# linhthi/BLISS-GNN

Measured on AMD Instinct MI355X. Metric: steps/sec (train step: sample_blocks + gather + SAGE fwd/bwd + Adam + exp3), reddit-like, higher is better.
Workload: dtype bf16

## Files before the change

bliss_gnn_amd/csrc/common.cuh:

```cuda
#pragma once
#include <hip/hip_runtime.h>
#include <stdint.h>
#include "bliss_gnn.h"

#define BLISS_WAVE 64

#define FRAC_DST 40
#define FRAC_SRC 44
#define FRAC_BLK 36

#define BLISS_ERR_CAP_FRONTIER 1
#define BLISS_ERR_CAP_CAND     2
#define BLISS_ERR_CAP_KEPT     4
#define BLISS_ERR_CAP_EDGES    8
#define BLISS_ERR_NONFINITE   16
#define BLISS_ERR_FIXED_RANGE 32
#define BLISS_ERR_CAP_SEEDS   64
#define BLISS_ERR_RNG_STREAM 128
#define BLISS_ERR_FLAG_TIMEOUT 256

typedef uint16_t bf16_t;

__device__ __forceinline__ float bf2f(bf16_t b) { return __uint_as_float(((uint32_t)b) << 16); }

// ... 53 lines not shown
__device__ __forceinline__ long long bf_to_fixed_wide(bf16_t b, int frac, long long* lo, int* sticky, int* bad) {
  uint32_t e = (b >> 7) & 0xff, m = b & 0x7f;
  if (e == 255) { *bad |= BLISS_ERR_NONFINITE; return 0; }
  if (e == 0) e = 1; else m |= 0x80;
  const int shift = (int)e - 134 + frac;
  const bool neg = (b & 0x8000) != 0;
  if (shift >= 0) {
    if (shift > 55) { *bad |= BLISS_ERR_FIXED_RANGE; return 0; }
    const long long mag = (long long)((uint64_t)m << shift);
    return neg ? -mag : mag;
  }
  const int rs = -shift;
  const uint32_t top = rs >= 8 ? 0u : (m >> rs);
  const uint32_t r = rs >= 8 ? m : (m & ((1u << rs) - 1u));
  if (r) {
    long long l;
    if (rs <= 40) l = (long long)((uint64_t)r << (40 - rs));
    else {
      const int d = rs - 40;
      l = d >= 8 ? 0 : (long long)(r >> d);
      if (d >= 8 || (r & ((1u << d) - 1u))) *sticky = 1;
    }
    *lo += neg ? -l : l;
  }
  return neg ? -(long long)top : (long long)top;
}

__device__ __forceinline__ bf16_t fixed_wide_to_bf(int64_t hi, int64_t lo, int sticky, int frac, int* bad) {
  if (lo == 0 && !sticky) return fixed_to_bf(hi, frac, bad);
  __int128 t = ((__int128)hi << 40) + (__int128)lo;
  if (t == 0) return 0;
  const uint32_t sign = t < 0 ? 0x8000u : 0u;
  const unsigned __int128 mag = t < 0 ? (unsigned __int128)(-t) : (unsigned __int128)t;
  const uint64_t mh = (uint64_t)(mag >> 64), ml = (uint64_t)mag;
  const int msb = mh ? 127 - __clzll((long long)mh) : 63 - __clzll((long long)ml);
  const int f = frac + 40;
  auto round_shift = [&](int sh) -> uint64_t {
    if (sh <= 0) return (uint64_t)(mag << (-sh));
    if (sh > 126) return 0;
    uint64_t q = (uint64_t)(mag >> sh);
    const unsigned __int128 rem = mag & ((((unsigned __int128)1) << sh) - 1), half = ((unsigned __int128)1) << (sh - 1);
    if (rem > half || (rem == half && (sticky || (q & 1)))) q += 1;
    return q;
  };
  if (msb - f + 127 <= 0) return (bf16_t)(sign | (uint32_t)round_shift(f - 133));
  uint64_t q = round_shift(msb - 7);
  int e = msb - f + 127;
  if (q >= 256) { q >>= 1; e += 1; }
  if (e >= 255) { *bad |= BLISS_ERR_FIXED_RANGE; return 0; }
  return (bf16_t)(sign | ((uint32_t)e << 7) | ((uint32_t)q & 0x7f));
}

struct PlainRange { unsigned lo, span; };
__device__ __forceinline__ PlainRange bf_plain_range(int frac) {
  int e_lo = 134 - frac, e_hi = 189 - frac;
  if (e_hi > 254) e_hi = 254;
  PlainRange r;
  r.lo = e_lo <= 1 ? 0u : (unsigned)e_lo << 7;
  const unsigned end = e_hi < 1 ? 0u : (unsigned)(e_hi + 1) << 7;
  r.span = end > r.lo ? end - r.lo : 0u;
  return r;
}
__device__ __forceinline__ bool bf_is_plain(bf16_t b, PlainRange r) { return (unsigned)b - r.lo < r.span; }
__device__ __forceinline__ long long bf_fixed_plain(bf16_t b, int frac) {
  const unsigned ef = (unsigned)b >> 7, m = (b & 0x7fu) | (ef ? 0x80u : 0u);
  const int shift = (int)(ef ? ef : 1u) - 134 + frac;
  return (long long)((uint64_t)m << (shift & 63));
}

__device__ __forceinline__ int lane_id() { return threadIdx.x & (BLISS_WAVE - 1); }

__device__ __forceinline__ int64_t shfl_up_i64(int64_t v, int d) {
  int lo = __shfl_up((int)(v & 0xffffffffll), d), hi = __shfl_up((int)(v >> 32), d);
  return ((int64_t)hi << 32) | (uint32_t)lo;
}

template <int CTRL, int ROW_MASK>
__device__ __forceinline__ int dpp_mov0(int v) { return __builtin_amdgcn_update_dpp(0, v, CTRL, ROW_MASK, 0xf, false); }
template <int CTRL, int ROW_MASK>
__device__ __forceinline__ long long dpp_mov0_i64(long long v) {
  const int lo = dpp_mov0<CTRL, ROW_MASK>((int)(v & 0xffffffffll)), hi = dpp_mov0<CTRL, ROW_MASK>((int)(v >> 32));
  return ((long long)hi << 32) | (unsigned)lo;
}
__device__ __forceinline__ int wave_total_i32(int v) {
  v += dpp_mov0<0x111, 0xf>(v); v += dpp_mov0<0x112, 0xf>(v); v += dpp_mov0<0x114, 0xf>(v); v += dpp_mov0<0x118, 0xf>(v);
  v += dpp_mov0<0x142, 0xa>(v); v += dpp_mov0<0x143, 0xc>(v);
  return __builtin_amdgcn_readlane(v, 63);
}
__device__ __forceinline__ int wave_max_u31(int v) {
  v = max(v, dpp_mov0<0x111, 0xf>(v)); v = max(v, dpp_mov0<0x112, 0xf>(v)); v = max(v, dpp_mov0<0x114, 0xf>(v));
  v = max(v, dpp_mov0<0x118, 0xf>(v)); v = max(v, dpp_mov0<0x142, 0xa>(v)); v = max(v, dpp_mov0<0x143, 0xc>(v));
  return __builtin_amdgcn_readlane(v, 63);
}
__device__ __forceinline__ int bf_exp_field(bf16_t b) { const int e = (b >> 7) & 0xff; return e == 0 ? 1 : e; }
__device__ __forceinline__ int rel_frac(int frac, int emax) { const int s = 126 - emax; return frac + (s > 0 ? s : 0); }

__device__ __forceinline__ long long wave_total_i64(long long v) {
  v += dpp_mov0_i64<0x111, 0xf>(v); v += dpp_mov0_i64<0x112, 0xf>(v); v += dpp_mov0_i64<0x114, 0xf>(v);
  v += dpp_mov0_i64<0x118, 0xf>(v); v += dpp_mov0_i64<0x142, 0xa>(v); v += dpp_mov0_i64<0x143, 0xc>(v);
  const int lo = __builtin_amdgcn_readlane((int)(v & 0xffffffffll), 63), hi = __builtin_amdgcn_readlane((int)(v >> 32), 63);
  return ((long long)hi << 32) | (unsigned)lo;
}
__device__ __forceinline__ bool wave_single_key(int key, int* k0) {
  const unsigned long long act = __ballot(key >= 0);
  if (!act) { *k0 = -1; return true; }
  *k0 = __builtin_amdgcn_readlane(key, __ffsll((long long)act) - 1);
  return __ballot(key >= 0 && key != *k0) == 0ull;
}

__device__ __forceinline__ void wave_segsum_atomic_i64(int key, int64_t v, unsigned long long* acc) {
  const int lane = lane_id();
  int k0;
  if (wave_single_key(key, &k0)) {
    if (k0 < 0) return;
    const long long tot = wave_total_i64(key >= 0 ? v : 0);
    if (lane == 0 && tot != 0) atomicAdd(acc + k0, (unsigned long long)tot);
    return;
  }
#pragma unroll
  for (int d = 1; d < BLISS_WAVE; d <<= 1) {
    int64_t vu = shfl_up_i64(v, d);
    int ku = __shfl_up(key, d);
    if (lane >= d && ku == key) v += vu;
  }
  int kn = __shfl_down(key, 1);
  if (key >= 0 && (lane == BLISS_WAVE - 1 || kn != key) && v != 0)
    atomicAdd(acc + key, (unsigned long long)v);
}
__device__ __forceinline__ void wave_segsum_atomic_i32(int key, int v, int* acc) {
  const int lane = lane_id();
  int k0;
  if (wave_single_key(key, &k0)) {
    if (k0 < 0) return;
    const int tot = wave_total_i32(key >= 0 ? v : 0);
    if (lane == 0 && tot != 0) atomicAdd(acc + k0, tot);
    return;
  }
#pragma unroll
  for (int d = 1; d < BLISS_WAVE; d <<= 1) {
    int vu = __shfl_up(v, d);
    int ku = __shfl_up(key, d);
    if (lane >= d && ku == key) v += vu;
  }
  int kn = __shfl_down(key, 1);
  if (key >= 0 && (lane == BLISS_WAVE - 1 || kn != key) && v != 0) atomicAdd(acc + key, v);
}

__device__ __forceinline__ int block_excl_scan(int v, int* sh, int* total) {
  const int lane = lane_id(), wid = threadIdx.x >> 6, nw = blockDim.x >> 6;
  int inc = v;
#pragma unroll
  for (int d = 1; d < BLISS_WAVE; d <<= 1) {
    int t = __shfl_up(inc, d);
    if (lane >= d) inc += t;
  }
  __syncthreads();
  if (lane == BLISS_WAVE - 1) sh[wid] = inc;
  __syncthreads();
  if (wid == 0) {
    int w = lane < nw ? sh[lane] : 0, winc = w;
#pragma unroll
    for (int d = 1; d < 16; d <<= 1) {
      int t = __shfl_up(winc, d);
      if (lane >= d) winc += t;
    }
    if (lane < nw) sh[lane] = winc - w;
    if (lane == nw - 1) sh[16] = winc;
  }
  __syncthreads();
  *total = sh[16];
  return sh[wid] + inc - v;
// ... 68 lines not shown
```

bliss_gnn_amd/csrc/sampler.hip:

```cpp
#include "common.cuh"
#include "bliss_gnn.h"
#include "prof.h"
#include "edge_q.cuh"
#include <cstdlib>

#ifndef TPB
#define TPB 256
#endif
#define ITEMS 4
#define CHUNK (TPB * ITEMS)

namespace {

#define SPAN (64 * ITEMS)
#define SEG_ZERO_WGS 8
#define LONG_COL 1024
#define LONG_FIRST 4096

struct alignas(8) ColEnt {
  int k, n;
  long long p0;
};

struct EdgeAt {
  int k;
  int64_t pos;
  int src;
};

__device__ __forceinline__ EdgeAt decode(int base, int E, int S, const int* __restrict__ seg_ptr,
                                         const long long* __restrict__ col_base, const int* __restrict__ indices, int* k_hint) {
  EdgeAt r;
  const int e = base + lane_id();
  r.k = wave_segment(seg_ptr, S, base, k_hint);
  r.pos = 0; r.src = 0;
  if (e < E) {
    r.pos = col_base[r.k] + e;
    r.src = indices[r.pos];
  } else r.k = -1;
  return r;
}

__device__ __forceinline__ int chunk_wave_offset(int wave_total, int* sh4, int* chunk_total) {
  const int wave = threadIdx.x >> 6;
  __syncthreads();
  if (lane_id() == 0) sh4[wave] = wave_total;
  __syncthreads();
  int off = 0, tot = 0;
#pragma unroll
  for (int w = 0; w < TPB / 64; ++w) { const int v = sh4[w]; tot += v; if (w < wave) off += v; }
  *chunk_total = tot;
  return off;
}

__device__ __forceinline__ void seg_scan_body(const int64_t* __restrict__ indptr, const int* __restrict__ seeds,
                                              LayerCounts* cnt, int S_host, const int* __restrict__ S_dev, int cap_s,
                                              unsigned long long* __restrict__ seed_acc, int* __restrict__ seg_ptr,
                                              int* __restrict__ local_id, int num_nodes, int* __restrict__ src_cnt, int cap_k,
                                              int* __restrict__ bin_cursor, int n_bins, long long* __restrict__ col_base,
                                              int* __restrict__ span_seg, long long frontier_cap, int* entry_flag,
                                              int wg, int n_wgs, bool keep_sums, int* sh, int* st_sh, ColEnt* long_list = nullptr) {
  if (entry_flag && wg == 0 && threadIdx.x == 0) __hip_atomic_store(entry_flag, 1, __ATOMIC_RELEASE, __HIP_MEMORY_SCOPE_AGENT);
  __shared__ int sh_long[2];
  if (long_list && threadIdx.x < 2) sh_long[threadIdx.x] = 0;
  int S = S_host >= 0 ? S_host : *S_dev;
  int bad = 0;
  if (S > cap_s) { S = cap_s; bad |= BLISS_ERR_CAP_SEEDS; }
  if (wg > 0 || n_wgs == 1) {
    const int nz = n_wgs > 1 ? n_wgs - 1 : 1, bz = n_wgs > 1 ? wg - 1 : 0;
    const int t0 = bz * blockDim.x + threadIdx.x, step = nz * blockDim.x;
    for (int i = (keep_sums ? 2 * cap_s : 0) + t0; i < cap_s * 5; i += step) seed_acc[i] = 0ull;
    if (src_cnt) for (int i = t0; i <= cap_k; i += step) src_cnt[i] = 0;
    if (bin_cursor) for (int i = t0; i <= n_bins; i += step) bin_cursor[i] = 0;
    for (int k = t0; k < S; k += step) { const int s = seeds[k]; if (s >= 0 && s < num_nodes) local_id[s] = k; }
    if (n_wgs > 1) return;
  }
  long long run = 0;
  constexpr int G = 4;
  for (int base0 = 0; base0 < S; base0 += G * (int)blockDim.x) {
    int degs[G];
    long long cols[G];
#pragma unroll
    for (int i = 0; i < G; ++i) {
      const int k = base0 + i * (int)blockDim.x + threadIdx.x;
      degs[i] = 0; cols[i] = 0;
      if (k < S) {
        const int s = seeds[k];
        if (s < 0 || s >= num_nodes) { bad |= BLISS_ERR_CAP_CAND; }
        else {
          cols[i] = indptr[s];
          degs[i] = (int)(indptr[s + 1] - cols[i]);
        }
      }
    }
#pragma unroll
    for (int i = 0; i < G; ++i) {
      const int k = base0 + i * (int)blockDim.x + threadIdx.x;
      if (base0 + i * (int)blockDim.x >= S) break;
      const int deg = degs[i];
      int tot, ex = block_excl_scan(deg, sh, &tot);
      const long long start = run + ex;
      if (k < S) {
        seg_ptr[k] = (int)start;
        col_base[k] = deg > 0 ? cols[i] - start : 0;
      }
      if (long_list) {
        const bool is_long = k < S && deg > LONG_COL, is_first = is_long && deg > LONG_FIRST;
        const unsigned long long m_first = __ballot(is_first), m_rest = __ballot(is_long && !is_first);
        if (m_first | m_rest) {
          int b_first = 0, b_rest = 0;
          if (lane_id() == 0) {
            if (m_first) b_first = atomicAdd(&sh_long[0], __popcll(m_first));
            if (m_rest) b_rest = atomicAdd(&sh_long[1], __popcll(m_rest));
          }
          b_first = __shfl(b_first, 0); b_rest = __shfl(b_rest, 0);
          if (is_long) {
            const unsigned long long below = (1ull << lane_id()) - 1ull;
            const int slot = is_first ? b_first + __popcll(m_first & below) : cap_s - 1 - (b_rest + __popcll(m_rest & below));
            ColEnt ent; ent.k = k; ent.n = deg; ent.p0 = cols[i];
            long_list[slot] = ent;
          }
        }
      }
      if (run + tot <= frontier_cap) {
        st_sh[threadIdx.x] = (int)(k < S ? start : run + tot);
        __syncthreads();
        const long long sp_end = (run + tot + SPAN - 1) / SPAN;
        for (long long sp = (run + SPAN - 1) / SPAN + threadIdx.x; sp < sp_end; sp += blockDim.x) {
          const int p = (int)(sp * SPAN);
          int t = 0;
#pragma unroll
          for (int step = 512; step >= 1; step >>= 1) if (st_sh[t + step] <= p) t += step;
          span_seg[sp] = base0 + i * (int)blockDim.x + t;
        }
      }
      run += tot;
      if (run > frontier_cap) bad |= BLISS_ERR_CAP_FRONTIER;
    }
  }
  int any_bad = __syncthreads_or(bad);
  if (threadIdx.x == 0) {
    if (long_list) { int* n_long = (int*)(long_list + cap_s); n_long[0] = sh_long[0]; n_long[1] = sh_long[1]; }
    seg_ptr[S] = (int)run;
    cnt->S = S; cnt->E = (any_bad & BLISS_ERR_CAP_FRONTIER) ? 0 : (int)run;
    cnt->C = 0; cnt->K = 0; cnt->B = 0; cnt->iters = 0; cnt->all_one = 0; cnt->c = 1.0;
    cnt->err = any_bad;
  }
}

__global__ void __launch_bounds__(1024) k_seg_scan(const int64_t* __restrict__ indptr, const int* __restrict__ seeds,
                                                   LayerCounts* cnt, int S_host, const int* __restrict__ S_dev, int cap_s,
                                                   unsigned long long* __restrict__ seed_acc, int* __restrict__ seg_ptr,
                                                   int* __restrict__ local_id, int num_nodes, int* __restrict__ src_cnt, int cap_k,
                                                   int* __restrict__ bin_cursor, int n_bins, long long* __restrict__ col_base,
                                                   int* __restrict__ span_seg, long long frontier_cap, int* entry_flag,
                                                   int keep_sums, ColEnt* long_list) {
// ... 387 lines not shown
      for (int r = 0; r < COL_RB; ++r) {
        const int i = t + r * COL_TPB;
        x[r] = 0;
        if (i < n) x[r] = wc[i];
      }
#pragma unroll
      for (int r = 0; r < COL_RB; ++r) wr.set(r, x[r]);
    }
#pragma unroll
    for (int r = 0; r < COL_RB; ++r)
      if (t + r * COL_TPB < n) emax = max(emax, bf_exp_field(wr.get(r)));
#pragma unroll 8
    for (int i = t + COL_RB * COL_TPB; i < n; i += COL_TPB) emax = max(emax, bf_exp_field(wc[i]));
    const int wfrac = rel_frac(FRAC_DST, block_max_u31<COL_TPB>(emax, sh));
    const PlainRange wr_ok = bf_plain_range(wfrac);
    bool odd = false;
#pragma unroll
    for (int r = 0; r < COL_RB; ++r)
      if (wave0 + r * COL_TPB < n) {
        odd |= t + r * COL_TPB < n && !bf_is_plain(wr.get(r), wr_ok);
        part += bf_fixed_plain(wr.get(r), wfrac);
      }
#pragma unroll 8
    for (int i = t + COL_RB * COL_TPB; i < n; i += COL_TPB) {
      const bf16_t b = wc[i];
      odd |= !bf_is_plain(b, wr_ok);
      part += bf_fixed_plain(b, wfrac);
    }
    long long lost;
    long long ws_fixed = block_sum2_i64<COL_TPB>(part, odd ? 1 : 0, sh2, &lost);
    bf16_t wsum;
    if (lost == 0) wsum = fixed_to_bf(ws_fixed, wfrac, &bad);
    else {
      long long part_lo = 0;
      int sticky = 0;
      part = 0;
#pragma unroll 4
      for (int i = t; i < n; i += COL_TPB) part += bf_to_fixed_wide(wc[i], wfrac, &part_lo, &sticky, &bad);
      ws_fixed = block_sum2_i64<COL_TPB>(part, (part_lo != 0 || sticky) ? 1 : 0, sh2, &lost);
      if (lost == 0) wsum = fixed_to_bf(ws_fixed, wfrac, &bad);
      else {
        const long long lo_tot = block_sum_i64<COL_TPB>(part_lo, sh);
        const long long st_tot = block_sum_i64<COL_TPB>(sticky, sh);
        wsum = fixed_wide_to_bf(ws_fixed, lo_tot, st_tot != 0, wfrac, &bad);
      }
    }
    const float a = rbf((1.0f / (float)n) * eta_f);
    const PlainRange q_ok = bf_plain_range(FRAC_DST);
    part = 0; odd = false;
#pragma unroll
    for (int r = 0; r < COL_RB; ++r)
      if (wave0 + r * COL_TPB < n) {
        const bool in = t + r * COL_TPB < n;
        const bf16_t q = edge_q_pre(wr.get(r), wsum, a, ome_f);
        odd |= in && !bf_is_plain(q, q_ok);
        part += in ? bf_fixed_plain(q, FRAC_DST) : 0ll;
      }
#pragma unroll 8
    for (int i = t + COL_RB * COL_TPB; i < n; i += COL_TPB) {
      const bf16_t q = edge_q_pre(wc[i], wsum, a, ome_f);
      odd |= !bf_is_plain(q, q_ok);
      part += bf_fixed_plain(q, FRAC_DST);
    }
    long long qs_fixed = block_sum2_i64<COL_TPB>(part, odd ? 1 : 0, sh2, &lost);
    if (lost != 0) {
      part = 0;
#pragma unroll 4
      for (int i = t; i < n; i += COL_TPB) part += bf_to_fixed(edge_q_pre(wc[i], wsum, a, ome_f), FRAC_DST, &bad);
      qs_fixed = block_sum_i64<COL_TPB>(part, sh);
    }
    if (t == 0) col_store(k, ws_fixed, qs_fixed, wsum, n, eta_f, acc_w, acc_q, seed_coef, &bad);
  }
  }
  if (bad) atomicOr(&cnt->err, bad);
}

template <bool BANDIT>
__global__ void __launch_bounds__(BIN_TPB) k_bin_scatter(const int64_t* __restrict__ indptr, const int* __restrict__ indices,
                                                     const bf16_t* __restrict__ w, const int* __restrict__ seeds,
                                                     const int* __restrict__ seg_ptr, const long long* __restrict__ col_base,
    const int* __restrict__ span_seg, LayerCounts* cnt,
                                                     const unsigned long long* __restrict__ acc_w,
                                                     const unsigned long long* __restrict__ acc_q, float eta_f, float ome_f,
                                                     int uniform_nodes, int n_bins, int log2_bins, long long bin_cap, int* bin_cursor,
                                                     unsigned long long* __restrict__ bin_rec, unsigned* __restrict__ bitmap,
                                                     const uint2* __restrict__ seed_coef) {
  __shared__ int hist[MAX_BINS];
  __shared__ int gbase[MAX_BINS];
  const int S = cnt->S, E = cnt->E, tid = threadIdx.x;
  const int nb = (E + BIN_BATCH - 1) / BIN_BATCH;
  const int bmask = n_bins - 1;
  int bad = 0;
  for (int batch = blockIdx.x; batch < nb; batch += gridDim.x) {
    for (int b = tid; b < n_bins; b += BIN_TPB) hist[b] = 0;
    if (tid < BIN_BATCH / 32) bitmap[batch * (BIN_BATCH / 32) + tid] = 0u;
    __syncthreads();
    int srcs[BIN_ITEMS], ranks[BIN_ITEMS];
    bf16_t ts[BIN_ITEMS];
    const int wbase = batch * BIN_BATCH + (tid >> 6) * (64 * BIN_ITEMS);
    int hint = span_seg[wbase >> 8];
#pragma unroll
    for (int j = 0; j < BIN_ITEMS; ++j) {
      ranks[j] = -1; srcs[j] = 0; ts[j] = 0;
      const int base = wbase + j * 64;
      if (base >= E) continue;
      EdgeAt a = decode(base, E, S, seg_ptr, col_base, indices, &hint);
      if (a.k >= 0) {
        bf16_t t;
        if (uniform_nodes) {
          t = (bf16_t)0x3f80;
        } else if (BANDIT) {
          const uint2 cf = seed_coef[a.k];
          bf16_t q = edge_q_pre(w[a.pos], (bf16_t)(cf.x & 0xffffu), __uint_as_float(cf.y), ome_f);
          float r = rbf(bf2f(q) / bf2f((bf16_t)(cf.x >> 16)));
          t = f2bf(r * r);
        } else {
          float x = bf2f(w[a.pos]);
          t = f2bf(x * x);
        }
        srcs[j] = a.src; ts[j] = t;
        ranks[j] = atomicAdd(&hist[a.src & bmask], 1);
      }
    }
    __syncthreads();
    for (int b = tid; b < n_bins; b += BIN_TPB) {
      const int h = hist[b];
      int g0 = 0;
      if (h) {
        g0 = atomicAdd(bin_cursor + b, h);
        if ((long long)g0 + h > bin_cap) bad |= BLISS_ERR_CAP_CAND;
      }
      gbase[b] = g0;
    }
    __syncthreads();
#pragma unroll
    for (int j = 0; j < BIN_ITEMS; ++j) {
      if (ranks[j] >= 0) {
        const int b = srcs[j] & bmask;
        const long long idx = (long long)gbase[b] + ranks[j];
        if (idx < bin_cap) {
          const size_t o = (size_t)b * (size_t)bin_cap + (size_t)idx;
          const unsigned e = (unsigned)(wbase + j * 64 + lane_id());
          bin_rec[o] = ((unsigned long long)e << 32) | ((unsigned long long)((unsigned)srcs[j] >> log2_bins) << 15) | (ts[j] & 0x7fffu);
        }
      }
    }
    __syncthreads();
  }
  if (bad) atomicOr(&cnt->err, bad);
}

__global__ void __launch_bounds__(BINRED_TPB) k_bin_reduce(LayerCounts* cnt, int n_bins, int log2_bins, long long bin_cap,
                                                           int* bin_cursor, const unsigned long long* __restrict__ bin_rec,
                                                           int num_nodes, int slots,
                                                           const int* __restrict__ local_id, unsigned long long* __restrict__ seed_p2,
                                                           unsigned long long* __restrict__ touched_key,
                                                           unsigned long long* __restrict__ touched_sum, unsigned* bitmap, int cap_c) {
  extern __shared__ unsigned long long dyn_lds[];
  unsigned long long* sm = dyn_lds;
  unsigned* mn = (unsigned*)(dyn_lds + slots);
  const int b = blockIdx.x, tid = threadIdx.x;
  if (cnt->E == 0) return;
  const int ne = b < num_nodes ? ((num_nodes - 1 - b) >> log2_bins) + 1 : 0;
  for (int i = tid; i < ne; i += BINRED_TPB) { sm[i] = 0ull; mn[i] = 0xffffffffu; }
  __syncthreads();
  long long n = bin_cursor[b];
  if (n > bin_cap) n = bin_cap;
  const unsigned long long* rec = bin_rec + (size_t)b * (size_t)bin_cap;
  int bad = 0;
  for (long long i = tid; i < n; i += BINRED_TPB) {
    const unsigned long long r = rec[i];
    const int li = (int)(((unsigned)r) >> 15);
    atomicMin(&mn[li], (unsigned)(r >> 32));
    const int64_t fx = bf_to_fixed((bf16_t)(r & 0x7fffu), FRAC_SRC, &bad);
    if (fx) atomicAdd(&sm[li], (unsigned long long)fx);
  }
  __syncthreads();
  __shared__ int wg_cnt, wg_base;
  if (tid == 0) wg_cnt = 0;
  __syncthreads();
  for (int li = tid; li < ne; li += BINRED_TPB) {
    bool is_cand = false;
    if (mn[li] != 0xffffffffu) {
      const int lid = local_id[((unsigned)li << log2_bins) | (unsigned)b];
      if (lid >= 0) { seed_p2[lid] = sm[li]; mn[li] = 0xffffffffu; }
      else is_cand = true;
    }
    const unsigned long long mask = __ballot(is_cand);
    if (mask && lane_id() == 0) atomicAdd(&wg_cnt, __popcll(mask));
  }
  __syncthreads();
  if (tid == 0) { wg_base = wg_cnt ? atomicAdd(bin_cursor + n_bins, wg_cnt) : 0; wg_cnt = 0; }
  __syncthreads();
  for (int li = tid; li < ne; li += BINRED_TPB) {
    const unsigned fp = mn[li];
    if (fp != 0xffffffffu) {
      const int j = wg_base + atomicAdd(&wg_cnt, 1);
      if (j < cap_c) { touched_key[j] = ((unsigned long long)fp << 32) | (((unsigned)li << log2_bins) | (unsigned)b); touched_sum[j] = sm[li]; }
      atomicOr(bitmap + (fp >> 5), 1u << (fp & 31u));
    }
  }
  if (bad) atomicOr(&cnt->err, bad);
}

#define BTILE_W 4
#define BTILE (1024 * BTILE_W)
#define MAX_TILES 2048
__global__ void __launch_bounds__(1024) k_bitmap_tiles(const unsigned* __restrict__ bitmap, int* __restrict__ word_prefix,
                                                       int* __restrict__ tile_sum, LayerCounts* cnt) {
  __shared__ int sh[17];
  const int nw = (cnt->E + 31) >> 5;
  const int ntiles = (nw + BTILE - 1) / BTILE;
  for (int tile = blockIdx.x; tile < ntiles; tile += gridDim.x) {
    const int i = tile * BTILE + threadIdx.x * BTILE_W;
    uint4 v = make_uint4(0, 0, 0, 0);
    if (i < nw) v = *reinterpret_cast<const uint4*>(bitmap + i);
    const int c0 = __popc(v.x), c1 = __popc(v.y), c2 = __popc(v.z), c3 = __popc(v.w);
    int total, ex = block_excl_scan(c0 + c1 + c2 + c3, sh, &total);
    if (i < nw) *reinterpret_cast<int4*>(word_prefix + i) = make_int4(ex, ex + c0, ex + c0 + c1, ex + c0 + c1 + c2);
    if (threadIdx.x == 0) tile_sum[tile] = total;
  }
}

__device__ __forceinline__ double block_sum_f64(double v, double* shd) {
  for (int d = 32; d >= 1; d >>= 1) {
    long long b = __double_as_longlong(v);
    int lo = __shfl_down((int)(b & 0xffffffffll), d), hi = __shfl_down((int)(b >> 32), d);
    v += __longlong_as_double(((long long)hi << 32) | (unsigned)lo);
  }
  __syncthreads();
  if (lane_id() == 0) shd[threadIdx.x >> 6] = v;
  __syncthreads();
  double t = 0;
  for (int i = 0; i < (int)(blockDim.x >> 6); ++i) t += shd[i];
  return t;
}

template <bool COHERENT>
__device__ __forceinline__ void poisson_scale_body(int* hist, LayerCounts* cnt, int C, int num, double eps, int* rng_ctl,
                                                   int* layer_off, int is_last, int rng_cap_total, int* __restrict__ sel_state,
                                                   double* shd) {
  for (int i = threadIdx.x; i < (C + CHUNK - 1) / CHUNK + 2; i += 1024) sel_state[i] = 0;
  if (rng_ctl && threadIdx.x == 1023) rng_stream_acquire(rng_ctl, C, layer_off, is_last, rng_cap_total);
  int n[HIST_BINS / 1024];
  bool any = false;
#pragma unroll
  for (int i = 0; i < HIST_BINS / 1024; ++i) {
    const int b = i * 1024 + threadIdx.x;
    n[i] = COHERENT ? __hip_atomic_load(hist + b, __ATOMIC_RELAXED, __HIP_MEMORY_SCOPE_AGENT) : hist[b];
  }
#pragma unroll
  for (int i = 0; i < HIST_BINS / 1024; ++i) {
    const int b = i * 1024 + threadIdx.x;
    if (n[i]) {
      if (COHERENT) __hip_atomic_store(hist + b, 0, __ATOMIC_RELAXED, __HIP_MEMORY_SCOPE_AGENT); else hist[b] = 0;
      any = true;
    }
  }
// ... 523 lines not shown
__global__ void __launch_bounds__(TPB) k_cleanup(LayerCounts* cnt, const int* __restrict__ cand_nid, int* local_id, int cap_c,
                                                 const int* __restrict__ kept_nid, int* kept_map, int cap_k) {
  maps_cleanup(cnt, cand_nid, local_id, cap_c, kept_nid, kept_map, cap_k);
}

inline int grid_for(int64_t n, int per_block, int max_blocks = 8192) {
  int64_t g = (n + per_block - 1) / per_block;
  if (g < 1) g = 1;
  if (g > max_blocks) g = max_blocks;
  return (int)g;
}

}

#define CK(x) do { hipError_t e_ = (x); if (e_ != hipSuccess) return (int)e_; } while (0)

static long long g_flag_spin_bound = 1ll << 22;
__global__ void __launch_bounds__(64) k_flag_wait(int* flag, int* err, long long bound) {
  if (threadIdx.x != 0) return;
  long long spins = 0;
  while (__hip_atomic_load(flag, __ATOMIC_RELAXED, __HIP_MEMORY_SCOPE_AGENT) == 0) {
    __builtin_amdgcn_s_sleep(8);
    if (++spins > bound) { if (err) atomicOr(err, BLISS_ERR_FLAG_TIMEOUT); break; }
  }
  __builtin_amdgcn_fence(__ATOMIC_ACQUIRE, "agent");
  __hip_atomic_store(flag, 0, __ATOMIC_RELAXED, __HIP_MEMORY_SCOPE_AGENT);
}

__global__ void k_flag_raise(int* flag) {
  if (threadIdx.x == 0) __hip_atomic_store(flag, 1, __ATOMIC_RELEASE, __HIP_MEMORY_SCOPE_AGENT);
}

extern "C" {

int bliss_layer_counts_bytes(void) { return (int)sizeof(LayerCounts); }

int bliss_flag_raise(int32_t* flag, void* stream) {
  if (!flag) return BLISS_EINVAL;
  k_flag_raise<<<1, 64, 0, (hipStream_t)stream>>>(flag);
  return (int)hipGetLastError();
}

int bliss_flag_wait(int32_t* flag, int32_t* err_word, void* stream) {
  if (!flag) return BLISS_EINVAL;
  k_flag_wait<<<1, 64, 0, (hipStream_t)stream>>>(flag, err_word, g_flag_spin_bound);
  return (int)hipGetLastError();
}

int bliss_flag_set_spin_bound(int64_t spins) {
  if (spins < 1) return BLISS_EINVAL;
  g_flag_spin_bound = spins;
  return 0;
}

int bliss_frontier_prob(const bliss_graph_t* g, const bliss_node_maps_t* m, const void* w_pos, const int32_t* seeds,
                        int32_t n_seeds, const int32_t* n_seeds_dev, int32_t cap_s, int mode, float eta_f,
                        float one_minus_eta_f, int64_t frontier_bound, const bliss_layer_ws_t* ws, void* stream_) {
  if (!g || !m || !seeds || !ws || !w_pos || cap_s <= 0 || !ws->hist || !ws->span_seg) return BLISS_EINVAL;
  if (n_seeds < 0 && !n_seeds_dev) return BLISS_EINVAL;
  if (n_seeds > cap_s) return BLISS_EINVAL;
  const int uniform_nodes = (mode & BLISS_MODE_UNIFORM_NODES) ? 1 : 0;
  const bool partials_only = (mode & BLISS_MODE_PARTIALS) != 0;
  mode &= ~(BLISS_MODE_UNIFORM_NODES | BLISS_MODE_PARTIALS);
  if (mode != BLISS_MODE_BANDIT && mode != BLISS_MODE_LADIES) return BLISS_EINVAL;
  if (partials_only && ws->n_bins <= 0) return BLISS_EINVAL;
  hipStream_t st = (hipStream_t)stream_;
  LayerCounts* cnt = (LayerCounts*)ws->counts;
  const bf16_t* w = (const bf16_t*)w_pos;
  unsigned long long* acc_w = (unsigned long long*)ws->seed_acc;
  unsigned long long* acc_q = acc_w + cap_s;
  const long long* col_base = (const long long*)(acc_w + 5 * (size_t)cap_s);
  if (frontier_bound < 1) frontier_bound = 1;
  const int ge = grid_for(frontier_bound, TPB), gc = grid_for(frontier_bound, CHUNK);
  const bool binned = ws->n_bins > 0;
  int log2_bins = 0, slots = 0;
  if (binned) {
    while ((1 << log2_bins) < ws->n_bins) ++log2_bins;
    slots = (g->num_nodes + ws->n_bins - 1) >> log2_bins;
    if ((1 << log2_bins) != ws->n_bins || ws->n_bins > MAX_BINS || (size_t)slots * 12 > 64 * 1024 || ws->bin_cap <= 0 ||
        g->num_edges > (long long)MAX_TILES * BTILE * 32 || !ws->bin_cursor || !ws->bin_rec || !ws->bitmap || !ws->word_prefix || !ws->touched_key || !ws->touched_sum)
      return BLISS_EINVAL;
  }
  const long long fcap = (long long)(g->num_edges < 0x7fffffffll ? g->num_edges : 0x7fffffffll);
  const bool col_sums = binned && mode == BLISS_MODE_BANDIT;
  ColEnt* long_list = (ColEnt*)(acc_w + 7 * (size_t)cap_s);
  PROF_LAUNCH(BK_SEG_SCAN, st, k_seg_scan<<<1 + SEG_ZERO_WGS, 1024, 0, st>>>(g->indptr, seeds, cnt, n_seeds, n_seeds_dev, cap_s, acc_w, ws->seg_ptr,
                                                            m->local_id, g->num_nodes, ws->src_cnt, ws->cap_k,
                                                            binned ? ws->bin_cursor : nullptr, ws->n_bins, (long long*)col_base, ws->span_seg,
                                                            fcap, ws->entry_flag, col_sums ? 1 : 0, col_sums ? long_list : nullptr));
  if (binned) {
    unsigned long long* seed_p2 = acc_w + 4 * (size_t)cap_s;
    uint2* seed_coef = (uint2*)(acc_w + 6 * (size_t)cap_s);
    unsigned long long* bin_rec = (unsigned long long*)ws->bin_rec;
    const int gb = grid_for(frontier_bound, BIN_BATCH);
    const int n_wave_wgs = (cap_s + COL_TPB / 64 - 1) / (COL_TPB / 64), n_block_wgs = cap_s < COL_BLOCK_WGS ? cap_s : COL_BLOCK_WGS;
    if (col_sums)
      PROF_LAUNCH(BK_COL_SUMS, st, k_col_sums<<<n_block_wgs + n_wave_wgs, COL_TPB, 0, st>>>(g->indptr, w, seeds, ws->seg_ptr, col_base, ws->span_seg, cnt, acc_w, acc_q, eta_f, one_minus_eta_f, seed_coef, n_block_wgs, long_list, cap_s));
    if (mode == BLISS_MODE_BANDIT)
      PROF_LAUNCH(BK_BIN_SCATTER, st, k_bin_scatter<true><<<gb, BIN_TPB, 0, st>>>(g->indptr, g->indices, w, seeds, ws->seg_ptr, col_base, ws->span_seg, cnt, acc_w, acc_q, eta_f, one_minus_eta_f, uniform_nodes, ws->n_bins, log2_bins, ws->bin_cap, ws->bin_cursor, bin_rec, ws->bitmap, seed_coef));
    else
      PROF_LAUNCH(BK_BIN_SCATTER, st, k_bin_scatter<false><<<gb, BIN_TPB, 0, st>>>(g->indptr, g->indices, w, seeds, ws->seg_ptr, col_base, ws->span_seg, cnt, acc_w, acc_q, eta_f, one_minus_eta_f, uniform_nodes, ws->n_bins, log2_bins, ws->bin_cap, ws->bin_cursor, bin_rec, ws->bitmap, seed_coef));
    PROF_LAUNCH(BK_BIN_REDUCE, st, k_bin_reduce<<<ws->n_bins, BINRED_TPB, (size_t)slots * 12, st>>>(
        cnt, ws->n_bins, log2_bins, ws->bin_cap, ws->bin_cursor, bin_rec, g->num_nodes, slots, m->local_id, seed_p2,
        (unsigned long long*)ws->touched_key, (unsigned long long*)ws->touched_sum, ws->bitmap, ws->cap_c));
    if (partials_only) return (int)hipGetLastError();
    int* tile_sum = ws->word_prefix;
    int* word_prefix = ws->word_prefix + MAX_TILES;
    PROF_LAUNCH(BK_BITMAP_SCAN, st, k_bitmap_tiles<<<grid_for(frontier_bound, (int64_t)BTILE * 32, MAX_TILES), 1024, 0, st>>>(ws->bitmap, word_prefix, tile_sum, cnt));
    int gf = (ws->cap_c + FIN_TPB - 1) / FIN_TPB;
    if (gf < 1) gf = 1;
    if (gf > 512) gf = 512;
    PROF_LAUNCH(BK_CAND_NUMBER, st, k_cand_number<<<gf, FIN_TPB, 0, st>>>(
        seeds, cnt, ws->cand_nid, m->local_id, seed_p2, (const unsigned long long*)ws->touched_key,
        (const unsigned long long*)ws->touched_sum, ws->bitmap, word_prefix, tile_sum, (bf16_t*)ws->p, ws->hist, ws->cap_c, uniform_nodes,
        FusedScale{ws->fs_ticket, ws->fs_fanout, ws->fs_eps, ws->fs_rng_ctl, ws->fs_layer_off, ws->fs_is_last, ws->fs_rng_cap, ws->chunk_cnt}));
    return (int)hipGetLastError();
  }
  if (mode == BLISS_MODE_BANDIT) {
    PROF_LAUNCH(BK_PASS1, st, k_frontier_pass1<true><<<ge, TPB, 0, st>>>(g->indptr, g->indices, w, seeds, ws->seg_ptr, col_base, ws->span_seg, cnt, m->local_id, m->first_pos, acc_w));
    PROF_LAUNCH(BK_PASS2, st, k_frontier_pass2<true><<<gc, TPB, 0, st>>>(g->indptr, g->indices, w, seeds, ws->seg_ptr, col_base, ws->span_seg, cnt, m->first_pos, acc_w, acc_q, ws->chunk_cnt, eta_f, one_minus_eta_f));
  } else {
    PROF_LAUNCH(BK_PASS1, st, k_frontier_pass1<false><<<ge, TPB, 0, st>>>(g->indptr, g->indices, w, seeds, ws->seg_ptr, col_base, ws->span_seg, cnt, m->local_id, m->first_pos, acc_w));
    PROF_LAUNCH(BK_PASS2, st, k_frontier_pass2<false><<<gc, TPB, 0, st>>>(g->indptr, g->indices, w, seeds, ws->seg_ptr, col_base, ws->span_seg, cnt, m->first_pos, acc_w, acc_q, ws->chunk_cnt, eta_f, one_minus_eta_f));
  }
  PROF_LAUNCH(BK_CHUNK_SCAN, st, k_chunk_scan<<<1, 1024, 0, st>>>(ws->chunk_cnt, cnt, 0, ws->cap_c));
  if (mode == BLISS_MODE_BANDIT)
    PROF_LAUNCH(BK_PASS3, st, k_frontier_pass3<true><<<gc, TPB, 0, st>>>(g->indptr, g->indices, w, seeds, ws->seg_ptr, col_base, ws->span_seg, cnt, m->first_pos, acc_w, acc_q, ws->chunk_cnt, m->local_id, ws->cand_nid, (unsigned long long*)m->acc_p2, eta_f, one_minus_eta_f, ws->cap_c, uniform_nodes));
  else
    PROF_LAUNCH(BK_PASS3, st, k_frontier_pass3<false><<<gc, TPB, 0, st>>>(g->indptr, g->indices, w, seeds, ws->seg_ptr, col_base, ws->span_seg, cnt, m->first_pos, acc_w, acc_q, ws->chunk_cnt, m->local_id, ws->cand_nid, (unsigned long long*)m->acc_p2, eta_f, one_minus_eta_f, ws->cap_c, uniform_nodes));
  {
    int gf = (ws->cap_c + FIN_TPB * 8 - 1) / (FIN_TPB * 8);
    if (gf < 1) gf = 1;
    if (gf > 256) gf = 256;
    PROF_LAUNCH(BK_CAND_FINALIZE, st, k_cand_finalize<<<gf, FIN_TPB, 0, st>>>(
        seeds, cnt, ws->cand_nid, (unsigned long long*)m->acc_p2, m->first_pos, (bf16_t*)ws->p, ws->hist, ws->cap_c, uniform_nodes));
  }
  return (int)hipGetLastError();
}

int bliss_poisson_select(const bliss_layer_ws_t* ws, int32_t fanout, double eps, const float* uniforms,
                         int32_t* uniforms_offset_dev, int32_t* rng_ctl, int is_last, int32_t rng_cap_total,
                         int64_t cand_bound, void* stream_) {
  if (!ws || !uniforms || fanout < 0 || (rng_ctl && !uniforms_offset_dev)) return BLISS_EINVAL;
  hipStream_t st = (hipStream_t)stream_;
  LayerCounts* cnt = (LayerCounts*)ws->counts;
  if (cand_bound < 1) cand_bound = 1;
  if (cand_bound > ws->cap_c) cand_bound = ws->cap_c;
  if (!ws->fs_ticket)
    PROF_LAUNCH(BK_POISSON_SCALE, st, k_poisson_scale<<<1, 1024, 0, st>>>(ws->hist, cnt, fanout, eps, rng_ctl, uniforms_offset_dev, is_last, rng_cap_total, ws->chunk_cnt));
  PROF_LAUNCH(BK_SELECT2, st, k_select_fused<<<grid_for(cand_bound, CHUNK, 1 << 20), TPB, 0, st>>>(
      (const bf16_t*)ws->p, uniforms, uniforms_offset_dev, cnt, (bf16_t*)ws->P, ws->chunk_cnt, ws->cand_nid, ws->new_id, ws->kept_nid,
      (bf16_t*)ws->node_prob, ws->cap_c, ws->cap_k, ws->kept_map));
  return (int)hipGetLastError();
}

int bliss_poisson_scale(int32_t* hist, void* counts, int32_t fanout, double eps, int32_t* scratch, void* stream_) {
  if (!hist || !counts || !scratch || fanout < 0) return BLISS_EINVAL;
  hipStream_t st = (hipStream_t)stream_;
  PROF_LAUNCH(BK_POISSON_SCALE, st, k_poisson_scale<<<1, 1024, 0, st>>>(hist, (LayerCounts*)counts, fanout, eps, nullptr, nullptr, 0, 0, scratch));
  return (int)hipGetLastError();
}

int bliss_multinomial_select(const bliss_layer_ws_t* ws, const int32_t* chosen, int32_t n_chosen, void* stream_) {
  if (!ws || n_chosen < 0 || (n_chosen > 0 && !chosen)) return BLISS_EINVAL;
  hipStream_t st = (hipStream_t)stream_;
  LayerCounts* cnt = (LayerCounts*)ws->counts;
  const int gc = grid_for(ws->cap_c, CHUNK), ge = grid_for(ws->cap_c, TPB);
  k_mn_prepare<<<ge, TPB, 0, st>>>(cnt, (const bf16_t*)ws->p, (bf16_t*)ws->P, ws->new_id, ws->cap_c);
  if (n_chosen > 0) k_mn_mark<<<grid_for(n_chosen, TPB), TPB, 0, st>>>(cnt, chosen, n_chosen, ws->new_id, ws->cap_c);
  k_mn_select<false><<<gc, TPB, 0, st>>>(cnt, (const bf16_t*)ws->P, ws->chunk_cnt, ws->cand_nid, ws->new_id, ws->kept_nid, (bf16_t*)ws->node_prob, ws->cap_c, ws->cap_k, ws->kept_map);
  k_chunk_scan<<<1, 1024, 0, st>>>(ws->chunk_cnt, cnt, 1, ws->cap_k);
  k_mn_select<true><<<gc, TPB, 0, st>>>(cnt, (const bf16_t*)ws->P, ws->chunk_cnt, ws->cand_nid, ws->new_id, ws->kept_nid, (bf16_t*)ws->node_prob, ws->cap_c, ws->cap_k, ws->kept_map);
  return (int)hipGetLastError();
}

int bliss_multinomial_select_marked(const bliss_layer_ws_t* ws, void* stream_) {
  if (!ws || !ws->counts || !ws->p || !ws->P || !ws->new_id || !ws->cand_nid || !ws->chunk_cnt || !ws->kept_nid || !ws->node_prob ||
      ws->cap_c <= 0 || ws->cap_k <= 0)
    return BLISS_EINVAL;
  hipStream_t st = (hipStream_t)stream_;
  LayerCounts* cnt = (LayerCounts*)ws->counts;
  const int gc = grid_for(ws->cap_c, CHUNK), ge = grid_for(ws->cap_c, TPB);
  k_mn_copy_p<<<ge, TPB, 0, st>>>(cnt, (const bf16_t*)ws->p, (bf16_t*)ws->P, ws->cap_c);
  k_mn_select<false><<<gc, TPB, 0, st>>>(cnt, (const bf16_t*)ws->P, ws->chunk_cnt, ws->cand_nid, ws->new_id, ws->kept_nid, (bf16_t*)ws->node_prob, ws->cap_c, ws->cap_k, ws->kept_map);
  k_chunk_scan<<<1, 1024, 0, st>>>(ws->chunk_cnt, cnt, 1, ws->cap_k);
  k_mn_select<true><<<gc, TPB, 0, st>>>(cnt, (const bf16_t*)ws->P, ws->chunk_cnt, ws->cand_nid, ws->new_id, ws->kept_nid, (bf16_t*)ws->node_prob, ws->cap_c, ws->cap_k, ws->kept_map);
// ... 51 lines not shown
```

Before: 1492.

## Stage bin scatter per batch in LDS and index bins via per-batch table

The bin scatter kernel stops using global atomic cursors per bin. Each batch now does a block-local prefix over its bins, stages the records in LDS in bin-sorted order, writes them out contiguously with 16-byte stores, and records each bin's (start, count) in a per-bin/per-batch table. The reduce kernel then walks that table row for its bin, prefetching entries and reading the runs with sub-groups of lanes. This removes global atomic contention and scattered writes, but the reduce kernel now reads many short, strided runs, and capacity overflow checking moves to a host-side size check.

```diff
diff --git a/bliss_gnn_amd/csrc/common.cuh b/bliss_gnn_amd/csrc/common.cuh
--- a/bliss_gnn_amd/csrc/common.cuh
+++ b/bliss_gnn_amd/csrc/common.cuh
@@ -159,11 +159,12 @@
   const int lo = dpp_mov0<CTRL, ROW_MASK>((int)(v & 0xffffffffll)), hi = dpp_mov0<CTRL, ROW_MASK>((int)(v >> 32));
   return ((long long)hi << 32) | (unsigned)lo;
 }
-__device__ __forceinline__ int wave_total_i32(int v) {
+__device__ __forceinline__ int wave_incl_scan_i32(int v) {
   v += dpp_mov0<0x111, 0xf>(v); v += dpp_mov0<0x112, 0xf>(v); v += dpp_mov0<0x114, 0xf>(v); v += dpp_mov0<0x118, 0xf>(v);
   v += dpp_mov0<0x142, 0xa>(v); v += dpp_mov0<0x143, 0xc>(v);
-  return __builtin_amdgcn_readlane(v, 63);
-}
+  return v;
+}
+__device__ __forceinline__ int wave_total_i32(int v) { return __builtin_amdgcn_readlane(wave_incl_scan_i32(v), 63); }
 __device__ __forceinline__ int wave_max_u31(int v) {
   v = max(v, dpp_mov0<0x111, 0xf>(v)); v = max(v, dpp_mov0<0x112, 0xf>(v)); v = max(v, dpp_mov0<0x114, 0xf>(v));
   v = max(v, dpp_mov0<0x118, 0xf>(v)); v = max(v, dpp_mov0<0x142, 0xa>(v)); v = max(v, dpp_mov0<0x143, 0xc>(v));
diff --git a/bliss_gnn_amd/csrc/sampler.hip b/bliss_gnn_amd/csrc/sampler.hip
--- a/bliss_gnn_amd/csrc/sampler.hip
+++ b/bliss_gnn_amd/csrc/sampler.hip
@@ -71,7 +71,7 @@
     const int t0 = bz * blockDim.x + threadIdx.x, step = nz * blockDim.x;
     for (int i = (keep_sums ? 2 * cap_s : 0) + t0; i < cap_s * 5; i += step) seed_acc[i] = 0ull;
     if (src_cnt) for (int i = t0; i <= cap_k; i += step) src_cnt[i] = 0;
-    if (bin_cursor) for (int i = t0; i <= n_bins; i += step) bin_cursor[i] = 0;
+    if (bin_cursor && t0 == 0) bin_cursor[n_bins] = 0;
     for (int k = t0; k < S; k += step) { const int s = seeds[k]; if (s >= 0 && s < num_nodes) local_id[s] = k; }
     if (n_wgs > 1) return;
   }
@@ -625,17 +625,19 @@
     const int* __restrict__ span_seg, LayerCounts* cnt,
                                                      const unsigned long long* __restrict__ acc_w,
                                                      const unsigned long long* __restrict__ acc_q, float eta_f, float ome_f,
-                                                     int uniform_nodes, int n_bins, int log2_bins, long long bin_cap, int* bin_cursor,
-                                                     unsigned long long* __restrict__ bin_rec, unsigned* __restrict__ bitmap,
+                                                     int uniform_nodes, int n_bins, int log2_bins,
+                                                     unsigned long long* __restrict__ bin_rec, unsigned* __restrict__ bin_tab,
+                                                     long long tab_stride, unsigned* __restrict__ bitmap,
                                                      const uint2* __restrict__ seed_coef) {
   __shared__ int hist[MAX_BINS];
-  __shared__ int gbase[MAX_BINS];
+  __shared__ int wsum[BIN_TPB / 64];
+  __shared__ __attribute__((aligned(16))) unsigned long long stage[BIN_BATCH];
+  static_assert(MAX_BINS <= BIN_TPB, "one thread per bin takes the prefix over the bins");
   const int S = cnt->S, E = cnt->E, tid = threadIdx.x;
   const int nb = (E + BIN_BATCH - 1) / BIN_BATCH;
   const int bmask = n_bins - 1;
-  int bad = 0;
   for (int batch = blockIdx.x; batch < nb; batch += gridDim.x) {
-    for (int b = tid; b < n_bins; b += BIN_TPB) hist[b] = 0;
+    if (tid < n_bins) hist[tid] = 0;
     if (tid < BIN_BATCH / 32) bitmap[batch * (BIN_BATCH / 32) + tid] = 0u;
     __syncthreads();
     int srcs[BIN_ITEMS], ranks[BIN_ITEMS];
@@ -666,35 +668,46 @@
       }
     }
     __syncthreads();
-    for (int b = tid; b < n_bins; b += BIN_TPB) {
-      const int h = hist[b];
-      int g0 = 0;
-      if (h) {
-        g0 = atomicAdd(bin_cursor + b, h);
-        if ((long long)g0 + h > bin_cap) bad |= BLISS_ERR_CAP_CAND;
-      }
-      gbase[b] = g0;
+    const int gsh = log2_bins >= 3 ? log2_bins - 3 : 0;
+    const int bin = log2_bins >= 3 ? ((tid & ((1 << gsh) - 1)) << 3) | (tid >> gsh) : tid;
+    const int h = tid < n_bins ? hist[bin] : 0;
+    const int inc = wave_incl_scan_i32(h);
+    if (lane_id() == 63) wsum[tid >> 6] = inc;
+    __syncthreads();
+    int start = inc - h, total = 0;
+#pragma unroll
+    for (int wv = 0; wv < BIN_TPB / 64; ++wv) { const int v = wsum[wv]; total += v; if (wv < (tid >> 6)) start += v; }
+    if (tid < n_bins) {
+      hist[bin] = start;
+      bin_tab[(size_t)bin * (size_t)tab_stride + (size_t)batch] = (unsigned)start | ((unsigned)h << 16);
     }
     __syncthreads();
 #pragma unroll
     for (int j = 0; j < BIN_ITEMS; ++j) {
       if (ranks[j] >= 0) {
-        const int b = srcs[j] & bmask;
-        const long long idx = (long long)gbase[b] + ranks[j];
-        if (idx < bin_cap) {
-          const size_t o = (size_t)b * (size_t)bin_cap + (size_t)idx;
-          const unsigned e = (unsigned)(wbase + j * 64 + lane_id());
-          bin_rec[o] = ((unsigned long long)e << 32) | ((unsigned long long)((unsigned)srcs[j] >> log2_bins) << 15) | (ts[j] & 0x7fffu);
-        }
+        const unsigned e = (unsigned)(wbase + j * 64 + lane_id());
+        stage[hist[srcs[j] & bmask] + ranks[j]] =
+            ((unsigned long long)e << 32) | ((unsigned long long)((unsigned)srcs[j] >> log2_bins) << 15) | (ts[j] & 0x7fffu);
       }
     }
     __syncthreads();
-  }
-  if (bad) atomicOr(&cnt->err, bad);
-}
-
-__global__ void __launch_bounds__(BINRED_TPB) k_bin_reduce(LayerCounts* cnt, int n_bins, int log2_bins, long long bin_cap,
+    unsigned long long* out = bin_rec + (size_t)batch * BIN_BATCH;
+    for (int i = tid; 2 * i + 1 < total; i += BIN_TPB)
+      reinterpret_cast<ulonglong2*>(out)[i] = reinterpret_cast<const ulonglong2*>(stage)[i];
+    if (tid == 0 && (total & 1)) out[total - 1] = stage[total - 1];
+    __syncthreads();
+  }
+}
+
+#ifndef BINRED_U
+#define BINRED_U 4
+#endif
+#ifndef BINRED_LMUL
+#define BINRED_LMUL 2
+#endif
+__global__ void __launch_bounds__(BINRED_TPB) k_bin_reduce(LayerCounts* cnt, int n_bins, int log2_bins, int lsh,
                                                            int* bin_cursor, const unsigned long long* __restrict__ bin_rec,
+                                                           const unsigned* __restrict__ bin_tab, long long tab_stride,
                                                            int num_nodes, int slots,
                                                            const int* __restrict__ local_id, unsigned long long* __restrict__ seed_p2,
                                                            unsigned long long* __restrict__ touched_key,
@@ -703,20 +716,47 @@
   unsigned long long* sm = dyn_lds;
   unsigned* mn = (unsigned*)(dyn_lds + slots);
   const int b = blockIdx.x, tid = threadIdx.x;
-  if (cnt->E == 0) return;
+  const unsigned* row = bin_tab + (size_t)b * (size_t)tab_stride;
+  const int L = 1 << lsh, sub = tid & (L - 1), grp = tid >> lsh, R = BINRED_TPB >> lsh;
+  unsigned ent[BINRED_U];
+#pragma unroll
+  for (int u = 0; u < BINRED_U; ++u) { const int r = u * R + grp; ent[u] = row[r < tab_stride ? r : tab_stride - 1]; }
+  const int E = cnt->E;
+  if (E == 0) return;
+  const int nb = (E + BIN_BATCH - 1) / BIN_BATCH;
   const int ne = b < num_nodes ? ((num_nodes - 1 - b) >> log2_bins) + 1 : 0;
   for (int i = tid; i < ne; i += BINRED_TPB) { sm[i] = 0ull; mn[i] = 0xffffffffu; }
   __syncthreads();
-  long long n = bin_cursor[b];
-  if (n > bin_cap) n = bin_cap;
-  const unsigned long long* rec = bin_rec + (size_t)b * (size_t)bin_cap;
   int bad = 0;
-  for (long long i = tid; i < n; i += BINRED_TPB) {
-    const unsigned long long r = rec[i];
+  auto take = [&](unsigned long long r) {
     const int li = (int)(((unsigned)r) >> 15);
     atomicMin(&mn[li], (unsigned)(r >> 32));
     const int64_t fx = bf_to_fixed((bf16_t)(r & 0x7fffu), FRAC_SRC, &bad);
     if (fx) atomicAdd(&sm[li], (unsigned long long)fx);
+  };
+  for (int r0 = 0; r0 < nb; r0 += BINRED_U * R) {
+    unsigned long long rc[BINRED_U];
+#pragma unroll
+    for (int u = 0; u < BINRED_U; ++u) {
+      const int r = r0 + u * R + grp;
+      if (r >= nb) ent[u] = 0u;
+      const int at = (int)(ent[u] & 0xffffu) + sub;
+      rc[u] = bin_rec[(size_t)(r < nb ? r : nb - 1) * BIN_BATCH + (at < BIN_BATCH ? at : BIN_BATCH - 1)];
+    }
+    unsigned nxt[BINRED_U];
+#pragma unroll
+    for (int u = 0; u < BINRED_U; ++u) { const int r = r0 + (BINRED_U + u) * R + grp; nxt[u] = row[r < nb ? r : nb - 1]; }
+#pragma unroll
+    for (int u = 0; u < BINRED_U; ++u) {
+      const int n = (int)(ent[u] >> 16);
+      if (sub < n) take(rc[u]);
+      if (n > L) {
+        const unsigned long long* run = bin_rec + (size_t)(r0 + u * R + grp) * BIN_BATCH + (ent[u] & 0xffffu);
+        for (int i = sub + L; i < n; i += L) take(run[i]);
+      }
+    }
+#pragma unroll
+    for (int u = 0; u < BINRED_U; ++u) ent[u] = nxt[u];
   }
   __syncthreads();
   __shared__ int wg_cnt, wg_base;
@@ -1406,6 +1446,9 @@
       return BLISS_EINVAL;
   }
   const long long fcap = (long long)(g->num_edges < 0x7fffffffll ? g->num_edges : 0x7fffffffll);
+  const long long max_batches = fcap > 0 ? (fcap + BIN_BATCH - 1) / BIN_BATCH : 1, rec_words = max_batches * BIN_BATCH;
+  if (binned && (rec_words + ((long long)ws->n_bins * max_batches + 1) / 2 > (long long)ws->n_bins * ws->bin_cap || ((uintptr_t)ws->bin_rec & 15u)))
+    return BLISS_EINVAL;
   const bool col_sums = binned && mode == BLISS_MODE_BANDIT;
   ColEnt* long_list = (ColEnt*)(acc_w + 7 * (size_t)cap_s);
   PROF_LAUNCH(BK_SEG_SCAN, st, k_seg_scan<<<1 + SEG_ZERO_WGS, 1024, 0, st>>>(g->indptr, seeds, cnt, n_seeds, n_seeds_dev, cap_s, acc_w, ws->seg_ptr,
@@ -1416,16 +1459,19 @@
     unsigned long long* seed_p2 = acc_w + 4 * (size_t)cap_s;
     uint2* seed_coef = (uint2*)(acc_w + 6 * (size_t)cap_s);
     unsigned long long* bin_rec = (unsigned long long*)ws->bin_rec;
+    unsigned* bin_tab = (unsigned*)(bin_rec + rec_words);
+    int lsh = 2;
+    while (lsh < 6 && (1 << lsh) < BINRED_LMUL * BIN_BATCH / ws->n_bins) ++lsh;
     const int gb = grid_for(frontier_bound, BIN_BATCH);
     const int n_wave_wgs = (cap_s + COL_TPB / 64 - 1) / (COL_TPB / 64), n_block_wgs = cap_s < COL_BLOCK_WGS ? cap_s : COL_BLOCK_WGS;
     if (col_sums)
       PROF_LAUNCH(BK_COL_SUMS, st, k_col_sums<<<n_block_wgs + n_wave_wgs, COL_TPB, 0, st>>>(g->indptr, w, seeds, ws->seg_ptr, col_base, ws->span_seg, cnt, acc_w, acc_q, eta_f, one_minus_eta_f, seed_coef, n_block_wgs, long_list, cap_s));
     if (mode == BLISS_MODE_BANDIT)
-      PROF_LAUNCH(BK_BIN_SCATTER, st, k_bin_scatter<true><<<gb, BIN_TPB, 0, st>>>(g->indptr, g->indices, w, seeds, ws->seg_ptr, col_base, ws->span_seg, cnt, acc_w, acc_q, eta_f, one_minus_eta_f, uniform_nodes, ws->n_bins, log2_bins, ws->bin_cap, ws->bin_cursor, bin_rec, ws->bitmap, seed_coef));
+      PROF_LAUNCH(BK_BIN_SCATTER, st, k_bin_scatter<true><<<gb, BIN_TPB, 0, st>>>(g->indptr, g->indices, w, seeds, ws->seg_ptr, col_base, ws->span_seg, cnt, acc_w, acc_q, eta_f, one_minus_eta_f, uniform_nodes, ws->n_bins, log2_bins, bin_rec, bin_tab, max_batches, ws->bitmap, seed_coef));
     else
-      PROF_LAUNCH(BK_BIN_SCATTER, st, k_bin_scatter<false><<<gb, BIN_TPB, 0, st>>>(g->indptr, g->indices, w, seeds, ws->seg_ptr, col_base, ws->span_seg, cnt, acc_w, acc_q, eta_f, one_minus_eta_f, uniform_nodes, ws->n_bins, log2_bins, ws->bin_cap, ws->bin_cursor, bin_rec, ws->bitmap, seed_coef));
+      PROF_LAUNCH(BK_BIN_SCATTER, st, k_bin_scatter<false><<<gb, BIN_TPB, 0, st>>>(g->indptr, g->indices, w, seeds, ws->seg_ptr, col_base, ws->span_seg, cnt, acc_w, acc_q, eta_f, one_minus_eta_f, uniform_nodes, ws->n_bins, log2_bins, bin_rec, bin_tab, max_batches, ws->bitmap, seed_coef));
     PROF_LAUNCH(BK_BIN_REDUCE, st, k_bin_reduce<<<ws->n_bins, BINRED_TPB, (size_t)slots * 12, st>>>(
-        cnt, ws->n_bins, log2_bins, ws->bin_cap, ws->bin_cursor, bin_rec, g->num_nodes, slots, m->local_id, seed_p2,
+        cnt, ws->n_bins, log2_bins, lsh, ws->bin_cursor, bin_rec, bin_tab, max_batches, g->num_nodes, slots, m->local_id, seed_p2,
         (unsigned long long*)ws->touched_key, (unsigned long long*)ws->touched_sum, ws->bitmap, ws->cap_c));
     if (partials_only) return (int)hipGetLastError();
     int* tile_sum = ws->word_prefix;
diff --git a/scratch/layer_medians.py b/scratch/layer_medians.py
--- /dev/null
+++ b/scratch/layer_medians.py
@@ -0,0 +1,29 @@
+import csv, sys, statistics as st
+path, label = sys.argv[1], sys.argv[2]
+rows = []
+with open(path) as f:
+    for r in csv.DictReader(f):
+        rows.append((int(r["Start_Timestamp"]), int(r["End_Timestamp"]), r["Kernel_Name"]))
+rows.sort()
+out = []
+for key in ("k_bin_scatter", "k_bin_reduce", "k_bitmap_tiles", "k_col_sums", "k_cand_number", "k_seg_scan"):
+    d = [(e - s) / 1e3 for s, e, n in rows if key in n]
+    d = d[len(d) % 3:]
+    d = d[-84 * 3:]
+    per = [round(st.median(d[i::3]), 2) for i in range(3)] if len(d) >= 3 else []
+    out.append("%s %s sum %.2f" % (key, per, sum(per)))
+spans, i = [], 0
+while i < len(rows):
+    if "k_exp3_update_multi" in rows[i][2]:
+        s0, n, j = rows[i][0], 0, i + 1
+        while j < len(rows) and n < 3 and "k_exp3_update_multi" not in rows[j][2]:
+            if "k_select_fused" in rows[j][2]:
+                n += 1
+                if n == 3:
+                    spans.append((rows[j][1] - s0) / 1e3)
+            j += 1
+        i = j
+    else:
+        i += 1
+spans = spans[-84:]
+print(label, " | ".join(out), "| span %.2f (n=%d)" % (st.median(spans) if spans else -1, len(spans)))
```

Result: no change. 1480 (-0.8%).
